# Kelvin-ywc/LPI

Measured on AMD Instinct MI355X. Metric: image-text pairs/sec fwd+bwd (ViT-B/16, bs256/GPU), higher is better.
Workload: dtype bf16; 1 GPU; BASELINE.json configs[2]: ViT-B/16 dual encoder bs=256/GPU prompt_depth=3 r=4 P=16, fwd+bwd incl. DecomposedPrompt grads + SGD step; global_batch=256, image=224x224, towers=lock step, GEMMs of one layer op grouped in one launch, parallelism=dp1, weights=synthetic (numpy Philox, CLIP-init scales), frozen

## Files before the change

### lpi_amd/csrc/gemm256p.hip

```cpp
#include "gemm256x128_tile.h"

extern int g_lpi_tuning[16];

namespace {

constexpr int T256 = 256;
constexpr int ROWB = 128;
constexpr int HALF_BYTES = 128 * ROWB;
constexpr int BUF_BYTES = 4 * HALF_BYTES;
constexpr int NTHR = 512;
constexpr int OFF_A0 = 0, OFF_A1 = HALF_BYTES, OFF_B0 = 2 * HALF_BYTES, OFF_B1 = 3 * HALF_BYTES;
constexpr int STG = BUF_BYTES;
constexpr int LDS_P = 2 * BUF_BYTES;
constexpr int EPI_PLAIN16 = 100;
template <int EPI, bool SAVE_U> constexpr bool slices_ok() { return !(EPI == LPI_EPI_QUICKGELU && SAVE_U); }

struct PProb {
    const void* A; const void* B; void* C; const float* bias; const void* residual; void* aux;
    int N, K, lda, ldb, ldc, ldr, ldaux, tiles_m, tiles_n;
    int vb0;
    int bias_off;
    int group_m;
};
struct PGroup {
    PProb p[2];
    int nprob;
    int n_full;
    int tail_blocks;
    int reserved;
    float alpha;
};

#ifdef LPI_GEMM_STAMPS
__device__ unsigned long long g_gemm_stamps[1024][8];
#define GS_NOW() __builtin_amdgcn_s_memtime()
#endif

template <typename T, typename TC, int EPI, bool RES, bool SAVE_U>
__global__ __launch_bounds__(NTHR, 2) void gemm256p_kernel(const PGroup grp)
{
    extern __shared__ __attribute__((aligned(16))) char smem[];
    constexpr int EPC = Elem<T>::EPC;
    constexpr int BK = ROWB / (int)sizeof(T);
    const int tid = threadIdx.x;
    const int lane = tid & 63;
    const int wave = __builtin_amdgcn_readfirstlane(tid >> 6);
    const int wm = wave >> 2, wn = wave & 3;
    const int G = gridDim.x;
    int group_m = 1;
    const float alpha = grp.alpha;
    typedef typename AuxT<T>::type TA;
    typedef float f32x8 __attribute__((ext_vector_type(8)));
    constexpr bool LNE = EPI == LPI_EPI_LN || EPI == LPI_EPI_LN_QUICKGELU;
    constexpr bool SLICES = slices_ok<EPI, SAVE_U>();
    constexpr bool P16 = EPI == EPI_PLAIN16;
    constexpr int EPIX = P16 ? LPI_EPI_NONE : EPI;
    const T* A = nullptr; const T* B = nullptr; TC* C = nullptr;
    const float* bias = nullptr; const float* residual = nullptr; TA* aux = nullptr;
    int K = 0, lda = 0, ldb = 0, ldc = 0, ldr = 0, ldaux = 0, tiles_m = 1, tiles_n = 1, nwg = 0, vb0 = 0, bias_off = 0;
    unsigned a_off = 0, b_off = 0;
    const int srow = tid >> 3;
    const int schunk = (tid & 7) ^ ((tid >> 4) & 7);
    auto bind = [&](int pi) {
        const PProb& P = grp.p[pi];
        A = (const T*)P.A; B = (const T*)P.B; C = (TC*)P.C; bias = P.bias; residual = (const float*)P.residual; aux = (TA*)P.aux;
        K = P.K; lda = P.lda; ldb = P.ldb; ldc = P.ldc; ldr = P.ldr; ldaux = P.ldaux; tiles_m = P.tiles_m; tiles_n = P.tiles_n;
        nwg = tiles_m * tiles_n; vb0 = P.vb0; bias_off = P.bias_off; group_m = P.group_m;
        a_off = (unsigned)(((size_t)srow * lda + schunk * EPC) * sizeof(T));
        b_off = (unsigned)(((size_t)srow * ldb + schunk * EPC) * sizeof(T));
    };

    auto coords = [&](int vb, int& m0, int& n0) {
        const int q = nwg >> 3, r = nwg & 7, xcd = vb & 7, idx = vb >> 3;
        const int t = (xcd < r ? xcd * (q + 1) : r * (q + 1) + (xcd - r) * q) + idx;
        const int gm = SLICES ? (group_m & 0xffff) : group_m;
        const int group = t / (gm * tiles_n);
        const int first_m = group * gm;
        const int gsz = min(tiles_m - first_m, gm);
        const int in_group = t - group * gm * tiles_n;
        m0 = (first_m + in_group % gsz) * T256;
        n0 = (in_group / gsz) * T256;
        if constexpr (SLICES) {
            const int wrap = (group_m >> 16) * T256;
            if (wrap) {
                if (m0 >= wrap) { m0 -= wrap; n0 += tiles_n * T256; }
                if (m0 >= wrap) { m0 -= wrap; n0 += tiles_n * T256; }
            }
        }
    };

    const unsigned lds_w = __builtin_amdgcn_readfirstlane((unsigned)(uintptr_t)(__attribute__((address_space(3))) char*)smem + wave * 1024);
    auto glds16 = [&](const T* sbase, unsigned voff, unsigned lds_addr) {
        unsigned keep;
        asm volatile("s_mov_b32 %0, m0\n\ts_mov_b32 m0, %3\n\ts_nop 0\n\tglobal_load_lds_dwordx4 %1, %2\n\ts_mov_b32 m0, %0"
                     : "=&s"(keep) : "v"(voff), "s"(sbase), "s"(lds_addr) : "memory");
    };
#ifndef LPI_A_POLICY
#define LPI_A_POLICY ""
#endif
    auto glds16a = [&](const T* sbase, unsigned voff, unsigned lds_addr) {
        unsigned keep;
        asm volatile("s_mov_b32 %0, m0\n\ts_mov_b32 m0, %3\n\ts_nop 0\n\tglobal_load_lds_dwordx4 %1, %2" LPI_A_POLICY "\n\ts_mov_b32 m0, %0"
                     : "=&s"(keep) : "v"(voff), "s"(sbase), "s"(lds_addr) : "memory");
    };
    auto stage_A = [&](int m0, int kt, int h, int buf) {
        const T* sb = A + (size_t)(m0 + h * 128) * lda + (size_t)kt * BK;
        const int lo = buf * BUF_BYTES + (h ? OFF_A1 : OFF_A0);
        glds16a(sb, a_off, lds_w + lo);
        glds16a(sb + (size_t)64 * lda, a_off, lds_w + lo + 8192);
    };
    auto stage_B = [&](int n0, int kt, int h, int buf) {
        const T* sb = B + (size_t)(n0 + h * 128) * ldb + (size_t)kt * BK;
        const int lo = buf * BUF_BYTES + (h ? OFF_B1 : OFF_B0);
        glds16(sb, b_off, lds_w + lo);
        glds16(sb + (size_t)64 * ldb, b_off, lds_w + lo + 8192);
    };

    const int frow = lane & 15, fg = lane >> 4, fsw = frow >> 1;
    int foff[2];
#pragma unroll
    for (int ks = 0; ks < 2; ++ks) foff[ks] = frow * ROWB + (((ks << 2) | fg) ^ fsw) * 16;
    const int a_base = (wm * 64) * ROWB;
    const int b_base = (wn * 32) * ROWB;

    Chunk fa[4][2], fb0[2][2], fb1[2][2];
    f32x4 acc[2][2][2][4];
    auto read_A = [&](const char* half) {
#pragma unroll
        for (int mi = 0; mi < 4; ++mi)
#pragma unroll
            for (int ks = 0; ks < 2; ++ks) fa[mi][ks].u = *reinterpret_cast<const uint4*>(half + a_base + mi * 16 * ROWB + foff[ks]);
    };
    auto read_B = [&](Chunk (&fb)[2][2], const char* half) {
#pragma unroll
        for (int ni = 0; ni < 2; ++ni)
#pragma unroll
            for (int ks = 0; ks < 2; ++ks) fb[ni][ks].u = *reinterpret_cast<const uint4*>(half + b_base + ni * 16 * ROWB + foff[ks]);
    };
    auto mma_quadrant = [&](f32x4 (&c)[2][2][2][4], int nh, int mh, const Chunk (&fb)[2][2]) {
        __builtin_amdgcn_s_setprio(1);
#pragma unroll
        for (int ks = 0; ks < 2; ++ks)
#pragma unroll
            for (int ni = 0; ni < 2; ++ni)
#pragma unroll
                for (int mi = 0; mi < 4; ++mi) mma_chunk<T>(c[nh][ni][mh][mi], fb[ni][ks], fa[mi][ks]);
        __builtin_amdgcn_s_setprio(0);
    };
#define PHASE_SYNC_IN()                                   \
    asm volatile("s_waitcnt lgkmcnt(0)" ::: "memory");    \
    __builtin_amdgcn_s_barrier();                         \
    __builtin_amdgcn_sched_barrier(0)
#define PHASE_SYNC_OUT()                                  \
    __builtin_amdgcn_sched_barrier(0);                    \
    __builtin_amdgcn_s_barrier();                         \
    asm volatile("" ::: "memory")

    int nk = 0;
    constexpr bool LATE = RES || EPI == LPI_EPI_DQUICKGELU;
    constexpr bool SIDE16 = (RES && sizeof(TC) == 2) || EPI == LPI_EPI_DQUICKGELU;
    constexpr bool STATS = EPI == LPI_EPI_NONE && RES && SAVE_U && __is_same(TC, f16_t);
    constexpr int NST = 8 + (STATS ? 2 : 0);
    const char* side_base = nullptr;
    int side_ld = 0;
    float* const bias_lds = reinterpret_cast<float*>(smem + LDS_P);
    if constexpr (SIDE16) {
        for (int pi = 0; pi < grp.nprob; ++pi) {
            const float* bp = grp.p[pi].bias;
            float* dst = bias_lds + grp.p[pi].bias_off;
            for (int i = tid * 4; i < grp.p[pi].N; i += NTHR * 4)
                *reinterpret_cast<f32x4*>(dst + i) = bp ? *reinterpret_cast<const f32x4*>(bp + i) : f32x4{0.f, 0.f, 0.f, 0.f};
        }
        __syncthreads();
    }
    auto stage_side = [&](int m0, int n0, int p) {
        const char* sb = side_base + ((size_t)m0 * side_ld + n0) * 2;
        int l2 = lane;
        asm volatile("" : "+v"(l2));
#pragma unroll
        for (int i = 0; i < 4; ++i) {
            const int sr = 2 * (4 * wave + i) + (l2 >> 5);
            const int trow = (p >> 1) * 128 + (sr >> 5) * 64 + ((p & 1) * 2 + ((sr >> 4) & 1)) * 16 + (sr & 15);
            const unsigned voff = (unsigned)trow * (unsigned)side_ld * 2u + (unsigned)(l2 & 31) * 16u;
            unsigned keep;
            asm volatile("s_mov_b32 %0, m0\n\ts_mov_b32 m0, %3\n\ts_nop 0\n\tglobal_load_lds_dwordx4 %1, %2 nt\n\ts_mov_b32 m0, %0"
                         : "=&s"(keep) : "v"(voff), "s"(sb), "s"(lds_w + (p & 1) * 32768 + i * 1024 + wave * 3072) : "memory");
        }
    };

#ifdef LPI_GEMM_STAMPS
    unsigned long long gs_main = 0, gs_epi = 0, gs_next = 0, gs_tiles = 0, gs_t0 = 0, gs_t1 = 0, gs_t2 = 0;
    unsigned long long gs_e[4] = {0, 0, 0, 0}, gs_a = 0, gs_b = 0;
#endif
    const int n_full = grp.n_full;
    int vbv = blockIdx.x;
    bool lds_used = false;
    for (int pi = 0; pi < grp.nprob; ++pi) {
        bind(pi);
        nk = K / BK;
        if constexpr (SIDE16) {
            side_base = RES ? reinterpret_cast<const char*>(residual) : reinterpret_cast<const char*>(aux);
            side_ld = RES ? ldr : ldaux;
        }
        const int vend = min(vb0 + nwg, n_full);
        if (vbv < vb0) vbv += (vb0 - vbv + G - 1) / G * G;
        if (vbv >= vend) continue;
        if (lds_used) {
            asm volatile("s_waitcnt lgkmcnt(0)" ::: "memory");
            __builtin_amdgcn_s_barrier();
            asm volatile("" ::: "memory");
        }
        lds_used = true;
        int vb = vbv - vb0;
        const int lend = vend - vb0;
        int m0, n0;
        coords(vb, m0, n0);
        m0 = __builtin_amdgcn_readfirstlane(m0);
        n0 = __builtin_amdgcn_readfirstlane(n0);
        stage_A(m0, 0, 0, 0); stage_B(n0, 0, 0, 0); stage_B(n0, 0, 1, 0); stage_A(m0, 0, 1, 0);
        stage_A(m0, 1, 0, 1); stage_B(n0, 1, 0, 1); stage_B(n0, 1, 1, 1);
        asm volatile("s_waitcnt vmcnt(8)" ::: "memory");
        __builtin_amdgcn_s_barrier();
        bool first = true;
        for (;;) {
            const int nvb = vb + G;
            const bool more_tiles = nvb < lend;
            const bool has_next = more_tiles && !LATE;
            int nm0 = 0, nn0 = 0;
            if (more_tiles) coords(nvb, nm0, nn0);
            nm0 = __builtin_amdgcn_readfirstlane(nm0);
            nn0 = __builtin_amdgcn_readfirstlane(nn0);
#pragma unroll
            for (int a = 0; a < 2; ++a)
#pragma unroll
                for (int b = 0; b < 2; ++b)
#pragma unroll
                    for (int c = 0; c < 2; ++c)
#pragma unroll
                        for (int d = 0; d < 4; ++d) acc[a][b][c][d] = f32x4{0.f, 0.f, 0.f, 0.f};
            if (wm == 1) __builtin_amdgcn_s_barrier();

            auto ktile = [&](int kt, const int BUF, bool skip_wait) {
                const char* buf = smem + BUF * BUF_BYTES;
                const bool more1 = kt + 1 < nk, more2 = kt + 2 < nk;
                read_B(fb0, buf + OFF_B0);
                read_B(fb1, buf + OFF_B1);
                __builtin_amdgcn_sched_barrier(0);
                read_A(buf + OFF_A0);
                if (more1) {
                    stage_A(m0, kt + 1, 1, BUF ^ 1);
                    if (!skip_wait) asm volatile("s_waitcnt vmcnt(8)" ::: "memory");
                } else if (has_next) {
                    stage_A(nm0, 0, 1, BUF ^ 1);
                    asm volatile("s_waitcnt vmcnt(8)" ::: "memory");
                } else {
                    asm volatile("s_waitcnt vmcnt(0)" ::: "memory");
                    if constexpr (SIDE16) {
                        stage_side(m0, n0, 0);
                        stage_side(m0, n0, 1);
                    }
                }
                PHASE_SYNC_IN();
                mma_quadrant(acc, 0, 0, fb0);
                mma_quadrant(acc, 1, 0, fb1);
                PHASE_SYNC_OUT();
                read_A(buf + OFF_A1);
                if (more2) {
                    stage_A(m0, kt + 2, 0, BUF); stage_B(n0, kt + 2, 0, BUF); stage_B(n0, kt + 2, 1, BUF);
                    asm volatile("s_waitcnt vmcnt(8)" ::: "memory");
                } else if (more1) {
                    if (has_next) {
                        stage_A(nm0, 0, 0, BUF); stage_B(nn0, 0, 0, BUF); stage_B(nn0, 0, 1, BUF);
                        asm volatile("s_waitcnt vmcnt(8)" ::: "memory");
                    } else {
                        asm volatile("s_waitcnt vmcnt(2)" ::: "memory");
                    }
                } else if (!has_next && !SIDE16) {
                    asm volatile("s_waitcnt vmcnt(0)" ::: "memory");
                }
                PHASE_SYNC_IN();
                mma_quadrant(acc, 1, 1, fb1);
                mma_quadrant(acc, 0, 1, fb0);
                PHASE_SYNC_OUT();
            };
#ifdef LPI_GEMM_STAMPS
            gs_t0 = GS_NOW();
            if (gs_tiles) gs_next += gs_t0 - gs_t2;
#endif
            ktile(0, 0, !first);
            ktile(1, 1, false);
            for (int kt = 2; kt < nk; kt += 2) {
                ktile(kt, 0, false);
                ktile(kt + 1, 1, false);
            }
            if (wm == 0) __builtin_amdgcn_s_barrier();
#ifdef LPI_GEMM_STAMPS
            gs_t1 = GS_NOW();
            gs_main += gs_t1 - gs_t0;
#endif

            int lane_e = lane, wave_e = wave;
            asm volatile("" : "+v"(lane_e));
            asm volatile("" : "+s"(wave_e));
            const int lrow = lane_e & 15, lslot = lane_e >> 4;
            const int wm_e = wave_e >> 2, wn_e = wave_e & 3;
            if constexpr (P16) {
                typedef __attribute__((ext_vector_type(4))) unsigned u32x4_;
                const int l5 = lane_e & 31, lh = lane_e >> 5;
                TC* const cbase = C + (size_t)m0 * ldc + n0 + l5 * 8;
#pragma unroll
                for (int p = 0; p < 4; ++p) {
                    const int mh = p >> 1;
                    char* const sb = smem + STG + (p & 1) * 32768;
#pragma unroll
                    for (int mi2 = 0; mi2 < 2; ++mi2) {
                        const int s_row = wm_e * 32 + mi2 * 16 + lrow;
#pragma unroll
                        for (int nh = 0; nh < 2; ++nh)
#pragma unroll
                            for (int ni = 0; ni < 2; ++ni) {
                                const int c8 = nh * 32 + wn_e * 8 + ni * 4 + lslot;
                                const f32x4 a = acc[nh][ni][mh][(p & 1) * 2 + mi2] + 0.0f;
                                *reinterpret_cast<uint2*>(sb + s_row * 512 + ((c8 ^ (2 * lrow)) << 3)) = uint2{pack2_t<TC>(a[0], a[1]), pack2_t<TC>(a[2], a[3])};
                            }
                    }
                    asm volatile("s_waitcnt lgkmcnt(0)" ::: "memory");
                    __builtin_amdgcn_s_barrier();
                    asm volatile("" ::: "memory");
#pragma unroll
                    for (int i = 0; i < 4; ++i) {
                        const int s_row = wave_e * 8 + 2 * i + lh;
                        const int trow = mh * 128 + (s_row >> 5) * 64 + ((p & 1) * 2 + ((s_row >> 4) & 1)) * 16 + (s_row & 15);
                        const u32x4_ v = *reinterpret_cast<const u32x4_*>(sb + s_row * 512 + (((2 * l5) ^ (2 * (s_row & 15))) << 3));
                        if constexpr (LPI_NTC_DEFAULT) __builtin_nontemporal_store(v, reinterpret_cast<u32x4_*>(cbase + (size_t)trow * ldc));
                        else *reinterpret_cast<u32x4_*>(cbase + (size_t)trow * ldc) = v;
                    }
                    if (p == 1 && has_next) asm volatile("s_waitcnt vmcnt(8)" ::: "memory");
                }
            } else {
            const int ecol = n0 + lane_e * 4;
            f32x4 bv = f32x4{0.f, 0.f, 0.f, 0.f};
            if constexpr (SIDE16) bv = *reinterpret_cast<const f32x4*>(bias_lds + bias_off + ecol);
            else if (bias) bv = *reinterpret_cast<const f32x4*>(bias + ecol);
            f32x4 c1v = f32x4{0.f, 0.f, 0.f, 0.f};
            if constexpr (EPI == LPI_EPI_LN || EPI == LPI_EPI_LN_QUICKGELU) c1v = *reinterpret_cast<const f32x4*>(residual + 2 * (size_t)ldr + ecol);
            char* const stg = smem + STG;
#pragma unroll
            for (int p = 0; p < 4; ++p) {
                const int mh = p >> 1;
#ifdef LPI_GEMM_STAMPS
                gs_a = GS_NOW();
#endif
                if (p) {
                    asm volatile("s_waitcnt lgkmcnt(0)" ::: "memory");
                    __builtin_amdgcn_s_barrier();
                }
#ifdef LPI_GEMM_STAMPS
                gs_b = GS_NOW(); gs_e[0] += gs_b - gs_a;
#endif
                if constexpr (SIDE16) {
                    if (p >= 1 && p <= 2) stage_side(m0, n0, p + 1);
                    if (p == 3 && more_tiles) { stage_A(nm0, 0, 0, 0); stage_A(nm0, 0, 1, 0); }
                }
                f32x8 mu8, rs8;
                if constexpr (LNE) {
                    const int sr0 = wave_e * 8;
                    const int trow0 = mh * 128 + (sr0 >> 5) * 64 + ((p & 1) * 2 + ((sr0 >> 4) & 1)) * 16 + (sr0 & 15);
                    const float* pm = residual + (m0 + trow0);
                    const float* pr = pm + ldr;
                    asm volatile("s_load_dwordx8 %0, %2, 0x0\n\ts_load_dwordx8 %1, %3, 0x0" : "=&s"(mu8), "=&s"(rs8) : "s"(pm), "s"(pr));
                }
#pragma unroll
                for (int mi2 = 0; mi2 < 2; ++mi2) {
                    const int s_row = wm_e * 32 + mi2 * 16 + lrow;
#pragma unroll
                    for (int nh = 0; nh < 2; ++nh)
#pragma unroll
                        for (int ni = 0; ni < 2; ++ni) {
                            const int chunk = nh * 32 + wn_e * 8 + ni * 4 + lslot;
                            *reinterpret_cast<f32x4*>(stg + s_row * 1024 + ((chunk ^ (s_row & 7)) << 4)) = acc[nh][ni][mh][(p & 1) * 2 + mi2];
                        }
                }
                if constexpr (SIDE16) {
                    if (p == 0) asm volatile("s_waitcnt vmcnt(4)" ::: "memory");
                    else if (p == 3 && !more_tiles) asm volatile("s_waitcnt vmcnt(%0)" :: "n"(NST) : "memory");
                    else asm volatile("s_waitcnt vmcnt(%0)" :: "n"(NST + 4) : "memory");
                }
                if constexpr (LNE) asm volatile("s_waitcnt lgkmcnt(0)" : "+s"(mu8), "+s"(rs8) : : "memory");
                else asm volatile("s_waitcnt lgkmcnt(0)" ::: "memory");
#ifdef LPI_GEMM_STAMPS
                gs_a = GS_NOW(); gs_e[1] += gs_a - gs_b;
#endif
                __builtin_amdgcn_s_barrier();
                asm volatile("" ::: "memory");
#ifdef LPI_GEMM_STAMPS
                gs_b = GS_NOW(); gs_e[2] += gs_b - gs_a;
#endif
                float st_s[8], st_q[8];
#pragma unroll
                for (int rr = 0; rr < 8; ++rr) {
                    const int s_row = wave_e * 8 + rr;
                    const int trow = mh * 128 + (s_row >> 5) * 64 + ((p & 1) * 2 + ((s_row >> 4) & 1)) * 16 + (s_row & 15);
                    const f32x4 v = *reinterpret_cast<const f32x4*>(stg + s_row * 1024 + ((lane_e ^ (s_row & 7)) << 4));
                    if constexpr (SIDE16) {
                        f32x4 o = v * alpha + bv;
                        const char* sp = smem + (p & 1) * 32768 + s_row * 512 + lane_e * 8;
                        if constexpr (EPI == LPI_EPI_DQUICKGELU) {
                            const f32x4 u = Elem<TA>::ld4(reinterpret_cast<const TA*>(sp));
                            o *= u;
                        } else {
                            o += Elem<TC>::ld4(reinterpret_cast<const TC*>(sp));
                        }
                        if constexpr (STATS) {
                            const uint32_t w0 = pack2_t<f16_t>(o[0], o[1]), w1 = pack2_t<f16_t>(o[2], o[3]);
                            *reinterpret_cast<uint2*>(C + (size_t)(m0 + trow) * ldc + ecol) = uint2{w0, w1};
                            f16x4_sum_sumsq(w0, w1, st_s[rr], st_q[rr]);
                        } else {
                            if constexpr (LPI_NTC_DEFAULT && EPI == LPI_EPI_DQUICKGELU) st4_nt<TC>(C + (size_t)(m0 + trow) * ldc + ecol, o);
                            else Elem<TC>::st4(C + (size_t)(m0 + trow) * ldc + ecol, o);
                        }
                    } else {
                        gemm_epilogue_store<T, TC, EPI, RES, SAVE_U>(v, m0 + trow, ecol, C, ldc, bv, alpha, residual, ldr, aux, ldaux, c1v, LNE ? mu8[rr] : 0.f,
                                                                     LNE ? rs8[rr] : 1.f);
                    }
                }
                if constexpr (STATS) {
                    float so, qo;
                    rowstats8_half_reduce(st_s, st_q, lane_e, so, qo);
                    const int s_row = wave_e * 8 + ((lane_e >> 2) & 7);
                    const int trow = mh * 128 + (s_row >> 5) * 64 + ((p & 1) * 2 + ((s_row >> 4) & 1)) * 16 + (s_row & 15);
                    float* sp = reinterpret_cast<float*>(aux) + (size_t)(2 * ((n0 >> 7) + (lane_e >> 5))) * ldaux + (m0 + trow);
                    if ((lane_e & 3) == 0) { sp[0] = so; sp[ldaux] = qo; }
                }
#ifdef LPI_GEMM_STAMPS
                gs_a = GS_NOW(); gs_e[3] += gs_a - gs_b;
#endif
                if (p == 1 && has_next) asm volatile("s_waitcnt vmcnt(16)" ::: "memory");
                if constexpr (LATE && !SIDE16) {
                    if (p == 1 && more_tiles) {
                        stage_A(nm0, 0, 0, 0); stage_B(nn0, 0, 0, 0); stage_B(nn0, 0, 1, 0); stage_A(nm0, 0, 1, 0);
                    }
                    if (p == 3 && more_tiles) asm volatile("s_waitcnt vmcnt(16)" ::: "memory");
                }
            }
            }
#ifdef LPI_GEMM_STAMPS
            gs_t2 = GS_NOW();
            gs_epi += gs_t2 - gs_t1;
            ++gs_tiles;
#endif
            if (!more_tiles) { vbv = nvb + vb0; break; }
            asm volatile("s_waitcnt lgkmcnt(0)" ::: "memory");
            __builtin_amdgcn_s_barrier();
            asm volatile("" ::: "memory");
            vb = nvb; m0 = nm0; n0 = nn0;
            if constexpr (SIDE16) {
                stage_B(n0, 0, 0, 0); stage_B(n0, 0, 1, 0);
                stage_A(m0, 1, 0, 1); stage_B(n0, 1, 0, 1); stage_B(n0, 1, 1, 1);
                asm volatile("s_waitcnt vmcnt(6)" ::: "memory");
                __builtin_amdgcn_s_barrier();
            } else {
                stage_A(m0, 1, 0, 1); stage_B(n0, 1, 0, 1); stage_B(n0, 1, 1, 1);
                first = false;
            }
        }
    }
#undef PHASE_SYNC_IN
#undef PHASE_SYNC_OUT

#ifdef LPI_GEMM_STAMPS
    if (tid == 0 && blockIdx.x < 1024) {
        g_gemm_stamps[blockIdx.x][0] = gs_main; g_gemm_stamps[blockIdx.x][1] = gs_epi; g_gemm_stamps[blockIdx.x][2] = gs_next; g_gemm_stamps[blockIdx.x][3] = gs_tiles;
        for (int i = 0; i < 4; ++i) g_gemm_stamps[blockIdx.x][4 + i] = gs_e[i];
    }
#endif
    if (grp.tail_blocks > 0) {
        for (int j = blockIdx.x; j < grp.tail_blocks; j += G) {
            const int k = (j >> 4) * 8 + (j & 7), half = (j >> 3) & 1;
            const int v = n_full + k;
            const int pi = (grp.nprob > 1 && v >= grp.p[1].vb0) ? 1 : 0;
            bind(pi);
            const int lv = v - vb0;
            if (lv < 0 || lv >= nwg) continue;
            __syncthreads();
            int m0, n0;
            coords(lv, m0, n0);
            t128::tile<T, TC, EPIX, RES, SAVE_U>(m0, n0 + half * 128, K, A, lda, B, ldb, C, ldc, bias, residual, ldr, aux, ldaux, alpha, smem);
        }
    }
}

int cu_count_p() { return lpi_cu_count(); }

struct HostProb {
    int M, N, K;
    const void* A; int lda; const void* B; int ldb; void* C; int ldc; const float* bias; const float* residual; int ldr; void* aux; int ldaux;
};

template <typename T, typename TC, int EPI, bool RES, bool SAVE_U>
int launchp_impl(const HostProb* hp, int np, float alpha, hipStream_t s)
{
    constexpr bool SIDE16 = (RES && sizeof(TC) == 2) || EPI == LPI_EPI_DQUICKGELU;
    static_assert(EPI != EPI_PLAIN16 || (!RES && !SAVE_U && sizeof(TC) == 2), "EPI_PLAIN16: store-only, 2-byte output");
    const int ncu = cu_count_p();
    PGroup g = {};
    g.nprob = np;
    g.alpha = alpha;
    int v = 0, nsum = 0;
    for (int i = 0; i < np; ++i) {
        PProb& P = g.p[i];
        const HostProb& h = hp[i];
        P.A = h.A; P.B = h.B; P.C = h.C; P.bias = h.bias; P.residual = h.residual; P.aux = h.aux;
        P.N = h.N; P.K = h.K; P.lda = h.lda; P.ldb = h.ldb; P.ldc = h.ldc; P.ldr = h.ldr; P.ldaux = h.ldaux;
        P.tiles_m = h.M / T256; P.tiles_n = h.N / T256;
        P.vb0 = v;
        v += P.tiles_m * P.tiles_n;
        P.bias_off = nsum;
        P.group_m = g_lpi_tuning[4] > 0 ? g_lpi_tuning[4] : ((size_t)h.N * h.K * sizeof(T) <= ((size_t)5 << 20) ? 1 : 8);
        if (slices_ok<EPI, SAVE_U>() && P.group_m == 1 && g_lpi_tuning[15] >= 0 && P.tiles_m < 32768) {
            int S = 0;
            const size_t wbytes = (size_t)h.N * h.K * sizeof(T);
            if (g_lpi_tuning[15] > 0) S = g_lpi_tuning[15];
            else if (wbytes > ((size_t)3 << 20) && P.tiles_n % 2 == 0) S = 2;
            if ((S == 2 || S == 3) && P.tiles_n % S == 0 && P.tiles_n / S >= 2) {
                P.group_m |= P.tiles_m << 16;
                P.tiles_n /= S;
                P.tiles_m *= S;
            }
        }
        nsum += h.N;
    }
    if (SIDE16 && nsum > 8192) return LPI_ENOSYS;
    const int rem = v % ncu;
    g.n_full = v;
    if (g_lpi_tuning[6] != 0 && v - rem >= ncu && rem > 0 && rem <= ncu / 2 && (ncu % 8) == 0) {
        g.n_full = v - rem;
        g.tail_blocks = 16 * ((rem + 7) >> 3);
    }
    auto kern = gemm256p_kernel<T, TC, EPI, RES, SAVE_U>;
    const int LDS = std::max<int>(t128::LDS_BYTES, LDS_P + (SIDE16 ? nsum * 4 : 0));
    static LdsOnce once;
    if (int e = lpi_ensure_lds(once, (const void*)kern, 160 * 1024)) return e;
    lpi_note_gemm_kernel(g.tail_blocks ? LPI_GEMM_K_256_TAIL : LPI_GEMM_K_256);
    const int grid = std::min(ncu, std::max(g.n_full, g.tail_blocks));
    LPI_LAUNCH(kern, dim3(grid), dim3(NTHR), LDS, s, g);
    LPI_CHECK_LAST();
    return 0;
}

template <typename T, typename TC>
int dispatchp(int epi, const HostProb* hp, int np, float alpha, hipStream_t s)
{
    const bool res = hp[0].residual != nullptr, ax = hp[0].aux != nullptr;
    for (int i = 1; i < np; ++i)
        if ((hp[i].residual != nullptr) != res || (hp[i].aux != nullptr) != ax) return LPI_EINVAL;
    switch (epi) {
    case LPI_EPI_NONE:
        if (res) return launchp_impl<T, TC, LPI_EPI_NONE, true, false>(hp, np, alpha, s);
        if constexpr (sizeof(TC) == 2) {
            bool plain = alpha == 1.0f && !ax && g_lpi_tuning[14] != 1;
            for (int i = 0; i < np; ++i) plain = plain && hp[i].bias == nullptr;
            if (plain) return launchp_impl<T, TC, EPI_PLAIN16, false, false>(hp, np, alpha, s);
        }
        return launchp_impl<T, TC, LPI_EPI_NONE, false, false>(hp, np, alpha, s);
    case LPI_EPI_RES_ROWSTATS:
        if constexpr (sizeof(TC) == 2 && !__is_same(TC, bf16_t)) {
            if (!res || !ax) return LPI_EINVAL;
            return launchp_impl<T, TC, LPI_EPI_NONE, true, true>(hp, np, alpha, s);
        }
        return LPI_ENOSYS;
    case LPI_EPI_QUICKGELU:
        if (res) return LPI_ENOSYS;
        if (ax) return launchp_impl<T, TC, LPI_EPI_QUICKGELU, false, true>(hp, np, alpha, s);
        return launchp_impl<T, TC, LPI_EPI_QUICKGELU, false, false>(hp, np, alpha, s);
    case LPI_EPI_DQUICKGELU:
        if (res) return LPI_ENOSYS;
        if (!ax) return LPI_EINVAL;
        return launchp_impl<T, TC, LPI_EPI_DQUICKGELU, false, false>(hp, np, alpha, s);
    }
    return LPI_EINVAL;
}

template <typename T, typename TC>
int dispatchp_ln(int epi, const HostProb* hp, int np, float alpha, hipStream_t s)
{
    const bool ax = hp[0].aux != nullptr;
    for (int i = 0; i < np; ++i)
        if (!hp[i].residual || (hp[i].aux != nullptr) != ax) return LPI_EINVAL;
    if (epi == LPI_EPI_LN) {
        if (ax) return LPI_EINVAL;
        return launchp_impl<T, TC, LPI_EPI_LN, false, false>(hp, np, alpha, s);
    }
    if (ax) return launchp_impl<T, TC, LPI_EPI_LN_QUICKGELU, false, true>(hp, np, alpha, s);
    return launchp_impl<T, TC, LPI_EPI_LN_QUICKGELU, false, false>(hp, np, alpha, s);
}

int launch_group(int dtype, int c_dtype, int epilogue, const HostProb* hp, int np, float alpha, hipStream_t s)
{
    if (epilogue == LPI_EPI_LN || epilogue == LPI_EPI_LN_QUICKGELU) {
        if (dtype == LPI_F16 && c_dtype == LPI_BF16) return dispatchp_ln<f16_t, bf16_t>(epilogue, hp, np, alpha, s);
        if (dtype == LPI_F16 && c_dtype == LPI_F16) return dispatchp_ln<f16_t, f16_t>(epilogue, hp, np, alpha, s);
        if (dtype == LPI_BF16 && c_dtype == LPI_BF16) return dispatchp_ln<bf16_t, bf16_t>(epilogue, hp, np, alpha, s);
        return LPI_ENOSYS;
    }
    if (dtype == LPI_BF16 && c_dtype == LPI_BF16) return dispatchp<bf16_t, bf16_t>(epilogue, hp, np, alpha, s);
    if (dtype == LPI_BF16 && c_dtype == LPI_F32) return dispatchp<bf16_t, float>(epilogue, hp, np, alpha, s);
    if (dtype == LPI_BF16 && c_dtype == LPI_F16 && (epilogue == LPI_EPI_NONE || epilogue == LPI_EPI_RES_ROWSTATS) && hp[0].residual) {
        for (int i = 1; i < np; ++i) if (!hp[i].residual) return LPI_EINVAL;
        if (epilogue == LPI_EPI_RES_ROWSTATS) {
            for (int i = 0; i < np; ++i) if (!hp[i].aux) return LPI_EINVAL;
            return launchp_impl<bf16_t, f16_t, LPI_EPI_NONE, true, true>(hp, np, alpha, s);
        }
        return launchp_impl<bf16_t, f16_t, LPI_EPI_NONE, true, false>(hp, np, alpha, s);
    }
    if (dtype == LPI_F16 && c_dtype == LPI_F16) return dispatchp<f16_t, f16_t>(epilogue, hp, np, alpha, s);
    if (dtype == LPI_F16 && c_dtype == LPI_F32) return dispatchp<f16_t, float>(epilogue, hp, np, alpha, s);
    return LPI_ENOSYS;
}

}

#ifdef LPI_GEMM_STAMPS
extern "C" int lpi_gemm_stamps_read(unsigned long long* dst) {
    return (int)hipMemcpyFromSymbol(dst, HIP_SYMBOL(g_gemm_stamps), sizeof(unsigned long long) * 1024 * 8, 0, hipMemcpyDeviceToHost);
}
#endif

int lpi_gemm256p_launch(int dtype, int c_dtype, int M, int N, int K, const void* A, int lda, const void* B, int ldb, void* C, int ldc,
                        const float* bias, const float* residual, int ldr, int epilogue, void* aux, int ldaux, float alpha, hipStream_t s)
{
    const HostProb hp = {M, N, K, A, lda, B, ldb, C, ldc, bias, residual, ldr, aux, ldaux};
    return launch_group(dtype, c_dtype, epilogue, &hp, 1, alpha, s);
}

int lpi_gemm256p_launch2(int dtype, int c_dtype, int epilogue, float alpha, const lpi_gemm_desc* d, hipStream_t s)
{
    HostProb hp[2];
    for (int i = 0; i < 2; ++i)
        hp[i] = HostProb{d[i].M, d[i].N, d[i].K, d[i].A, d[i].lda, d[i].B, d[i].ldb, d[i].C, d[i].ldc, d[i].bias, (const float*)d[i].residual, d[i].ldr,
                         d[i].aux, d[i].ldaux};
    return launch_group(dtype, c_dtype, epilogue, hp, 2, alpha, s);
}
```

Baseline: 11920 pairs/s.

## Stage residual/aux side tiles into dedicated LDS region, overlapping with mainloop

```diff
diff --git a/lpi_amd/csrc/gemm256p.hip b/lpi_amd/csrc/gemm256p.hip
--- a/lpi_amd/csrc/gemm256p.hip
+++ b/lpi_amd/csrc/gemm256p.hip
@@ -12,6 +12,8 @@
 constexpr int OFF_A0 = 0, OFF_A1 = HALF_BYTES, OFF_B0 = 2 * HALF_BYTES, OFF_B1 = 3 * HALF_BYTES;
 constexpr int STG = BUF_BYTES;
 constexpr int LDS_P = 2 * BUF_BYTES;
+constexpr int SIDE = LDS_P;
+constexpr int SIDE_BYTES = 64 * 512;
 constexpr int EPI_PLAIN16 = 100;
 template <int EPI, bool SAVE_U> constexpr bool slices_ok() { return !(EPI == LPI_EPI_QUICKGELU && SAVE_U); }
 
@@ -19,7 +21,6 @@
     const void* A; const void* B; void* C; const float* bias; const void* residual; void* aux;
     int N, K, lda, ldb, ldc, ldr, ldaux, tiles_m, tiles_n;
     int vb0;
-    int bias_off;
     int group_m;
 };
 struct PGroup {
@@ -57,7 +58,7 @@
     constexpr int EPIX = P16 ? LPI_EPI_NONE : EPI;
     const T* A = nullptr; const T* B = nullptr; TC* C = nullptr;
     const float* bias = nullptr; const float* residual = nullptr; TA* aux = nullptr;
-    int K = 0, lda = 0, ldb = 0, ldc = 0, ldr = 0, ldaux = 0, tiles_m = 1, tiles_n = 1, nwg = 0, vb0 = 0, bias_off = 0;
+    int K = 0, lda = 0, ldb = 0, ldc = 0, ldr = 0, ldaux = 0, tiles_m = 1, tiles_n = 1, nwg = 0, vb0 = 0;
     unsigned a_off = 0, b_off = 0;
     const int srow = tid >> 3;
     const int schunk = (tid & 7) ^ ((tid >> 4) & 7);
@@ -65,7 +66,7 @@
         const PProb& P = grp.p[pi];
         A = (const T*)P.A; B = (const T*)P.B; C = (TC*)P.C; bias = P.bias; residual = (const float*)P.residual; aux = (TA*)P.aux;
         K = P.K; lda = P.lda; ldb = P.ldb; ldc = P.ldc; ldr = P.ldr; ldaux = P.ldaux; tiles_m = P.tiles_m; tiles_n = P.tiles_n;
-        nwg = tiles_m * tiles_n; vb0 = P.vb0; bias_off = P.bias_off; group_m = P.group_m;
+        nwg = tiles_m * tiles_n; vb0 = P.vb0; group_m = P.group_m;
         a_off = (unsigned)(((size_t)srow * lda + schunk * EPC) * sizeof(T));
         b_off = (unsigned)(((size_t)srow * ldb + schunk * EPC) * sizeof(T));
     };
@@ -157,36 +158,32 @@
     asm volatile("" ::: "memory")
 
     int nk = 0;
-    constexpr bool LATE = RES || EPI == LPI_EPI_DQUICKGELU;
     constexpr bool SIDE16 = (RES && sizeof(TC) == 2) || EPI == LPI_EPI_DQUICKGELU;
+    constexpr bool LATE = RES && !SIDE16;
     constexpr bool STATS = EPI == LPI_EPI_NONE && RES && SAVE_U && __is_same(TC, f16_t);
     constexpr int NST = 8 + (STATS ? 2 : 0);
     const char* side_base = nullptr;
     int side_ld = 0;
-    float* const bias_lds = reinterpret_cast<float*>(smem + LDS_P);
-    if constexpr (SIDE16) {
-        for (int pi = 0; pi < grp.nprob; ++pi) {
-            const float* bp = grp.p[pi].bias;
-            float* dst = bias_lds + grp.p[pi].bias_off;
-            for (int i = tid * 4; i < grp.p[pi].N; i += NTHR * 4)
-                *reinterpret_cast<f32x4*>(dst + i) = bp ? *reinterpret_cast<const f32x4*>(bp + i) : f32x4{0.f, 0.f, 0.f, 0.f};
-        }
-        __syncthreads();
-    }
-    auto stage_side = [&](int m0, int n0, int p) {
-        const char* sb = side_base + ((size_t)m0 * side_ld + n0) * 2;
+    auto stage_side = [&](int m0, int n0, int p, int i0, int i1) {
+        int l2 = lane, w2 = wave;
+        asm volatile("" : "+v"(l2));
+        asm volatile("" : "+s"(w2));
+        const int trow0 = (p >> 1) * 128 + (w2 >> 2) * 64 + ((p & 1) * 2 + ((w2 >> 1) & 1)) * 16 + (w2 & 1) * 8;
+        const char* sb = side_base + ((size_t)(m0 + trow0) * side_ld + n0) * 2;
+        const unsigned voff = (unsigned)(l2 >> 5) * (unsigned)side_ld * 2u + (unsigned)(l2 & 31) * 16u;
+#pragma unroll
+        for (int i = i0; i < i1; ++i) {
+            unsigned keep;
+            asm volatile("s_mov_b32 %0, m0\n\ts_mov_b32 m0, %3\n\ts_nop 0\n\tglobal_load_lds_dwordx4 %1, %2 nt\n\ts_mov_b32 m0, %0"
+                         : "=&s"(keep) : "v"(voff), "s"(sb + (size_t)(2 * i) * side_ld * 2), "s"(lds_w + SIDE + i * 1024 + w2 * 3072) : "memory");
+        }
+    };
+    auto load_bias = [&](f32x4& bv, int n0) {
         int l2 = lane;
         asm volatile("" : "+v"(l2));
-#pragma unroll
-        for (int i = 0; i < 4; ++i) {
-            const int sr = 2 * (4 * wave + i) + (l2 >> 5);
-            const int trow = (p >> 1) * 128 + (sr >> 5) * 64 + ((p & 1) * 2 + ((sr >> 4) & 1)) * 16 + (sr & 15);
-            const unsigned voff = (unsigned)trow * (unsigned)side_ld * 2u + (unsigned)(l2 & 31) * 16u;
-            unsigned keep;
-            asm volatile("s_mov_b32 %0, m0\n\ts_mov_b32 m0, %3\n\ts_nop 0\n\tglobal_load_lds_dwordx4 %1, %2 nt\n\ts_mov_b32 m0, %0"
-                         : "=&s"(keep) : "v"(voff), "s"(sb), "s"(lds_w + (p & 1) * 32768 + i * 1024 + wave * 3072) : "memory");
-        }
-    };
+        asm volatile("global_load_dwordx4 %0, %1, %2" : "+v"(bv) : "v"(l2 * 16), "s"(bias + n0) : "memory");
+    };
+#define VM_WAIT(n) asm volatile("s_waitcnt vmcnt(%0)" ::"n"(n) : "memory")
 
 #ifdef LPI_GEMM_STAMPS
     unsigned long long gs_main = 0, gs_epi = 0, gs_next = 0, gs_tiles = 0, gs_t0 = 0, gs_t1 = 0, gs_t2 = 0;
@@ -252,13 +249,11 @@
                     if (!skip_wait) asm volatile("s_waitcnt vmcnt(8)" ::: "memory");
                 } else if (has_next) {
                     stage_A(nm0, 0, 1, BUF ^ 1);
-                    asm volatile("s_waitcnt vmcnt(8)" ::: "memory");
+                    if constexpr (!SIDE16) VM_WAIT(8);
+                    else VM_WAIT(12);
                 } else {
-                    asm volatile("s_waitcnt vmcnt(0)" ::: "memory");
-                    if constexpr (SIDE16) {
-                        stage_side(m0, n0, 0);
-                        stage_side(m0, n0, 1);
-                    }
+                    if constexpr (!SIDE16) VM_WAIT(0);
+                    else VM_WAIT(4);
                 }
                 PHASE_SYNC_IN();
                 mma_quadrant(acc, 0, 0, fb0);
@@ -269,11 +264,16 @@
                     stage_A(m0, kt + 2, 0, BUF); stage_B(n0, kt + 2, 0, BUF); stage_B(n0, kt + 2, 1, BUF);
                     asm volatile("s_waitcnt vmcnt(8)" ::: "memory");
                 } else if (more1) {
+                    if constexpr (SIDE16) {
+                        stage_side(m0, n0, 0, 0, 4);
+                    }
                     if (has_next) {
                         stage_A(nm0, 0, 0, BUF); stage_B(nn0, 0, 0, BUF); stage_B(nn0, 0, 1, BUF);
-                        asm volatile("s_waitcnt vmcnt(8)" ::: "memory");
+                        if constexpr (!SIDE16) VM_WAIT(8);
+                        else VM_WAIT(12);
                     } else {
-                        asm volatile("s_waitcnt vmcnt(2)" ::: "memory");
+                        if constexpr (!SIDE16) VM_WAIT(2);
+                        else VM_WAIT(6);
                     }
                 } else if (!has_next && !SIDE16) {
                     asm volatile("s_waitcnt vmcnt(0)" ::: "memory");
@@ -340,8 +340,11 @@
             } else {
             const int ecol = n0 + lane_e * 4;
             f32x4 bv = f32x4{0.f, 0.f, 0.f, 0.f};
-            if constexpr (SIDE16) bv = *reinterpret_cast<const f32x4*>(bias_lds + bias_off + ecol);
-            else if (bias) bv = *reinterpret_cast<const f32x4*>(bias + ecol);
+            if constexpr (SIDE16) {
+                if constexpr (RES) if (bias) load_bias(bv, n0);
+            } else if (bias) {
+                bv = *reinterpret_cast<const f32x4*>(bias + ecol);
+            }
             f32x4 c1v = f32x4{0.f, 0.f, 0.f, 0.f};
             if constexpr (EPI == LPI_EPI_LN || EPI == LPI_EPI_LN_QUICKGELU) c1v = *reinterpret_cast<const f32x4*>(residual + 2 * (size_t)ldr + ecol);
             char* const stg = smem + STG;
@@ -358,10 +361,6 @@
 #ifdef LPI_GEMM_STAMPS
                 gs_b = GS_NOW(); gs_e[0] += gs_b - gs_a;
 #endif
-                if constexpr (SIDE16) {
-                    if (p >= 1 && p <= 2) stage_side(m0, n0, p + 1);
-                    if (p == 3 && more_tiles) { stage_A(nm0, 0, 0, 0); stage_A(nm0, 0, 1, 0); }
-                }
                 f32x8 mu8, rs8;
                 if constexpr (LNE) {
                     const int sr0 = wave_e * 8;
@@ -381,13 +380,23 @@
                             *reinterpret_cast<f32x4*>(stg + s_row * 1024 + ((chunk ^ (s_row & 7)) << 4)) = acc[nh][ni][mh][(p & 1) * 2 + mi2];
                         }
                 }
+                uint2 sv[4];
                 if constexpr (SIDE16) {
-                    if (p == 0) asm volatile("s_waitcnt vmcnt(4)" ::: "memory");
-                    else if (p == 3 && !more_tiles) asm volatile("s_waitcnt vmcnt(%0)" :: "n"(NST) : "memory");
-                    else asm volatile("s_waitcnt vmcnt(%0)" :: "n"(NST + 4) : "memory");
+                    if (p == 0) {
+                        if constexpr (RES) asm volatile("s_waitcnt vmcnt(0)" : "+v"(bv) : : "memory");
+                        else if (has_next) VM_WAIT(8);
+                        else VM_WAIT(0);
+                    } else {
+                        VM_WAIT(NST - 4);
+                    }
+#pragma unroll
+                    for (int rr = 0; rr < 4; ++rr) sv[rr] = *reinterpret_cast<const uint2*>(smem + SIDE + (wave_e * 8 + rr) * 512 + lane_e * 8);
                 }
                 if constexpr (LNE) asm volatile("s_waitcnt lgkmcnt(0)" : "+s"(mu8), "+s"(rs8) : : "memory");
                 else asm volatile("s_waitcnt lgkmcnt(0)" ::: "memory");
+                if constexpr (SIDE16) {
+                    if (p < 3) stage_side(m0, n0, p + 1, 0, 2);
+                }
 #ifdef LPI_GEMM_STAMPS
                 gs_a = GS_NOW(); gs_e[1] += gs_a - gs_b;
 #endif
@@ -398,13 +407,20 @@
 #endif
                 float st_s[8], st_q[8];
 #pragma unroll
-                for (int rr = 0; rr < 8; ++rr) {
+                for (int q = 0; q < 8; ++q) {
+                    const int rr = SIDE16 ? ((q + 4) & 7) : q;
+                    if constexpr (SIDE16) {
+                        if (q == 4 && p < 3) {
+                            asm volatile("s_waitcnt lgkmcnt(0)" ::: "memory");
+                            stage_side(m0, n0, p + 1, 2, 4);
+                        }
+                    }
                     const int s_row = wave_e * 8 + rr;
                     const int trow = mh * 128 + (s_row >> 5) * 64 + ((p & 1) * 2 + ((s_row >> 4) & 1)) * 16 + (s_row & 15);
                     const f32x4 v = *reinterpret_cast<const f32x4*>(stg + s_row * 1024 + ((lane_e ^ (s_row & 7)) << 4));
                     if constexpr (SIDE16) {
                         f32x4 o = v * alpha + bv;
-                        const char* sp = smem + (p & 1) * 32768 + s_row * 512 + lane_e * 8;
+                        const char* sp = rr < 4 ? reinterpret_cast<const char*>(&sv[rr & 3]) : smem + SIDE + s_row * 512 + lane_e * 8;
                         if constexpr (EPI == LPI_EPI_DQUICKGELU) {
                             const f32x4 u = Elem<TA>::ld4(reinterpret_cast<const TA*>(sp));
                             o *= u;
@@ -435,8 +451,10 @@
 #ifdef LPI_GEMM_STAMPS
                 gs_a = GS_NOW(); gs_e[3] += gs_a - gs_b;
 #endif
-                if (p == 1 && has_next) asm volatile("s_waitcnt vmcnt(16)" ::: "memory");
-                if constexpr (LATE && !SIDE16) {
+                if constexpr (!SIDE16) {
+                    if (p == 1 && has_next) asm volatile("s_waitcnt vmcnt(16)" ::: "memory");
+                }
+                if constexpr (LATE) {
                     if (p == 1 && more_tiles) {
                         stage_A(nm0, 0, 0, 0); stage_B(nn0, 0, 0, 0); stage_B(nn0, 0, 1, 0); stage_A(nm0, 0, 1, 0);
                     }
@@ -454,19 +472,13 @@
             __builtin_amdgcn_s_barrier();
             asm volatile("" ::: "memory");
             vb = nvb; m0 = nm0; n0 = nn0;
-            if constexpr (SIDE16) {
-                stage_B(n0, 0, 0, 0); stage_B(n0, 0, 1, 0);
-                stage_A(m0, 1, 0, 1); stage_B(n0, 1, 0, 1); stage_B(n0, 1, 1, 1);
-                asm volatile("s_waitcnt vmcnt(6)" ::: "memory");
-                __builtin_amdgcn_s_barrier();
-            } else {
-                stage_A(m0, 1, 0, 1); stage_B(n0, 1, 0, 1); stage_B(n0, 1, 1, 1);
-                first = false;
-            }
+            stage_A(m0, 1, 0, 1); stage_B(n0, 1, 0, 1); stage_B(n0, 1, 1, 1);
+            first = false;
         }
     }
 #undef PHASE_SYNC_IN
 #undef PHASE_SYNC_OUT
+#undef VM_WAIT
 
 #ifdef LPI_GEMM_STAMPS
     if (tid == 0 && blockIdx.x < 1024) {
@@ -506,7 +518,7 @@
     PGroup g = {};
     g.nprob = np;
     g.alpha = alpha;
-    int v = 0, nsum = 0;
+    int v = 0;
     for (int i = 0; i < np; ++i) {
         PProb& P = g.p[i];
         const HostProb& h = hp[i];
@@ -515,7 +527,6 @@
         P.tiles_m = h.M / T256; P.tiles_n = h.N / T256;
         P.vb0 = v;
         v += P.tiles_m * P.tiles_n;
-        P.bias_off = nsum;
         P.group_m = g_lpi_tuning[4] > 0 ? g_lpi_tuning[4] : ((size_t)h.N * h.K * sizeof(T) <= ((size_t)5 << 20) ? 1 : 8);
         if (slices_ok<EPI, SAVE_U>() && P.group_m == 1 && g_lpi_tuning[15] >= 0 && P.tiles_m < 32768) {
             int S = 0;
@@ -528,9 +539,7 @@
                 P.tiles_m *= S;
             }
         }
-        nsum += h.N;
-    }
-    if (SIDE16 && nsum > 8192) return LPI_ENOSYS;
+    }
     const int rem = v % ncu;
     g.n_full = v;
     if (g_lpi_tuning[6] != 0 && v - rem >= ncu && rem > 0 && rem <= ncu / 2 && (ncu % 8) == 0) {
@@ -538,7 +547,7 @@
         g.tail_blocks = 16 * ((rem + 7) >> 3);
     }
     auto kern = gemm256p_kernel<T, TC, EPI, RES, SAVE_U>;
-    const int LDS = std::max<int>(t128::LDS_BYTES, LDS_P + (SIDE16 ? nsum * 4 : 0));
+    const int LDS = std::max<int>(t128::LDS_BYTES, LDS_P + (SIDE16 ? SIDE_BYTES : 0));
     static LdsOnce once;
     if (int e = lpi_ensure_lds(once, (const void*)kern, 160 * 1024)) return e;
     lpi_note_gemm_kernel(g.tail_blocks ? LPI_GEMM_K_256_TAIL : LPI_GEMM_K_256);
```

Result: no change. 11930 pairs/s (median of 6 runs) (+0.1%).
